# ImIntheMiddle/VATL4Pose-WACV2024

Hardware: AMD Instinct MI355X
Metric: frames/sec pose-infer+uncertainty, 256x192 17-kp (higher is better)
Workload: dtype f32; 1 GPU; SimpleBaseline-R50 256x192 inference + decode + local-peak + THC-L1, 1024-frame synthetic video per GPU; frames_per_gpu=1024, batch=1024, tracks=4, parallelism=frame-sharded x1

## Files before the change

### include/vatl_hip.h

```cpp
#ifndef VATL_HIP_H
#define VATL_HIP_H

#include <stdint.h>

#ifdef __cplusplus
extern "C" {
#endif

#define VATL_VERSION 100
#define VATL_EINVAL  (-1)
#define VATL_ELAUNCH (-2)

int         vatl_version(void);
const char* vatl_last_error(void);

int vatl_flop_meter_begin(void);
int vatl_flop_meter_end(double* direct_flops, double* winograd_flops, int64_t* direct_launches, int64_t* winograd_launches);
#define VATL_ROUTE_NAMES "igemm,igemm_bnbwd,igemm_dma,persistent_1x1,streamk,rows_1x1,bottleneck_chain,stem_pool,halo_3x3," \
                         "winograd,winograd_2h,winograd_bnbwd,winograd_persist,winograd_c32,wgrad,winograd_wgrad,winograd_wgrad_2h," \
                         "winograd_wgrad_table,winograd_f4,winograd_f4_bnbwd,gemm1x1_ring,winograd_deconv43,winograd_s2_43,stem_pool_w1d," \
                         "chain_proj,chain_step"
int vatl_flop_meter_routes(int64_t* counts, int n);


int vatl_nchw_to_nhwc(const float* src, float* dst, int N, int C, int H, int W, int Cpad, void* stream);
int vatl_nhwc_to_nchw(const float* src, float* dst, int N, int C, int H, int W, void* stream);

int vatl_pack_conv_weight(const float* w_oihw, float* w_packed, int Cout, int Cin, int R, int S,
                          int CoutPad, int Spad, int CinPad, void* stream);
int vatl_pack_deconv4x4s2_weight(const float* w_iohw, float* w_packed, int Cin, int Cout, int CoutPad, void* stream);
int64_t vatl_stem_pool_weight_floats(void);
int vatl_pack_stem_pool_weight(const float* w_oihw, float* packed, void* stream);
int vatl_stem_pool_supported(int H, int W);
int vatl_stem7x7s2_pool_fwd(const float* x_nchw, const float* w_packed, const float* scale, const float* bias, float* y_nhwc,
                            int N, int H, int W, void* stream);
int64_t vatl_stem_pool_w1d_weight_floats(void);
int vatl_pack_stem_pool_w1d_weight(const float* w_oihw, float* packed, void* stream);
int vatl_stem_pool_w1d_supported(int H, int W);
int vatl_stem7x7s2_pool_w1d_fwd(const float* x_nchw, const float* w_packed, const float* scale, const float* bias, float* y_nhwc,
                                int N, int H, int W, void* stream);
int64_t vatl_stem3_weight_floats(void);
int vatl_pack_stem3_weight(const float* w_oihw, float* packed, void* stream);
int vatl_stem3x3s2_fwd(const float* x_nchw, const float* w_packed, const float* scale, const float* bias, float* y_nhwc,
                       int N, int H, int W, void* stream);

int vatl_bn_fold(const float* gamma, const float* beta, const float* mean, const float* var, const float* conv_bias,
                 float eps, float* scale, float* bias, int C, void* stream);


int vatl_pack_conv1x1_dual_weight(const float* w1, const float* scale1, const float* bias1, const float* w2, const float* scale2,
                                  const float* bias2, float* out, float* bias, int Cout, int C1, int C2, int CoutPad, void* stream);
int vatl_conv1x1_dual_fwd(const float* a, const float* x, const float* w, const float* bias, float* y, int N, int Ho, int Wo,
                          int C1, int H2, int W2, int C2, int stride2, int Cout, int CoutPad, int relu, void* stream);

int64_t vatl_winograd_c32_weight_floats(void);
int vatl_pack_winograd_c32_weight(const float* w, float* u, void* stream);
int vatl_conv3x3_winograd_c32_supported(int N, int H, int W, int Cin, int Cout);
int vatl_conv3x3_winograd_c32_fwd(const float* x, const float* u, const float* scale, const float* bias, const float* residual, float* y, int N, int H, int W,
                                  int relu, void* stream);

int64_t vatl_winograd_f4_weight_floats(int Cout, int Cin);
int vatl_pack_winograd_f4_weight(const float* w, float* u, int Cout, int Cin, int data_gradient, void* stream);
int vatl_conv3x3_winograd_f4_supported(int N, int H, int W, int Cin, int Cout);
int vatl_conv3x3_winograd_f4_fwd(const float* x, const float* u, const float* scale, const float* bias, const float* residual, float* y, int N, int H, int W,
                                 int Cin, int Cout, int relu, void* stream);
int64_t vatl_winograd_f4_stats_row_blocks(int64_t N, int H, int W);
int vatl_conv3x3_winograd_f4_fwd_stats(const float* x, const float* u, float* y, double* stats, int64_t* row_blocks_used, int N, int H, int W, int Cin, int Cout,
                                       void* stream);
int vatl_conv3x3_winograd_f4_fwd_bnbwd(const float* x, const float* u, const float* residual, float* y, int N, int H, int W, int Cin, int Cout, const float* bn_z,
                                       const float* bn_mask_y, const float* bn_scale, const float* bn_bias, const float* bn_mean, const float* bn_invstd,
                                       double* stats, int64_t* row_blocks_used, void* stream);

int vatl_conv1x1_rows_supported(int K1, int K2, int N, int64_t M);
int vatl_conv1x1_rows_fwd(const float* a, const float* x2, const float* w, const float* scale, const float* bias, const float* residual, float* y,
                          int64_t M, int K1, int K2, int N, int relu, void* stream);

int vatl_bottleneck_chain_supported(int Cmid, int Cout, int Cnext, int64_t M);
int vatl_bottleneck_chain_fwd(const float* a, const float* w3, const float* scale3, const float* bias3, const float* skip, float* t,
                              const float* w1, const float* scale1, const float* bias1, float* y1, int64_t M, int Cmid, int Cout,
                              int Cnext, void* stream);

int vatl_chain_proj_supported(int Cmid, int Cout, int Cnext, int64_t M);
int vatl_chain_proj_fwd(const float* a, const float* x2, const float* w, const float* scale, const float* bias, float* t, const float* w1,
                        const float* scale1, const float* bias1, float* y1, int64_t M, int Cmid, int Cout, int Cnext, int relu, void* stream);
int vatl_chain_step_supported(int Cmid, int Cout, int Cnext, int64_t M);
int vatl_chain_step_fwd(const float* a, const float* w3, const float* scale3, const float* bias3, const float* skip, float* t, const float* w1,
                        const float* scale1, const float* bias1, float* y1, int64_t M, int Cmid, int Cout, int Cnext, void* stream);

int vatl_tune_set(int knob, int value);
int vatl_set_splitk_workspace(float* workspace, int64_t floats);
int vatl_set_splitk_workspace_thread(float* workspace, int64_t floats);
int64_t vatl_streamk_workspace_bytes(void);
int vatl_set_streamk_workspace_thread(void* workspace, int64_t bytes);
int vatl_conv_cout_pad(int Cout);
int vatl_conv2d_fwd(const float* x, const float* w, const float* scale, const float* bias, const float* residual,
                    float* y, int N, int H, int W, int Cin, int Cout, int CoutPad, int R, int S, int stride, int pad,
                    int relu, int out_nchw, void* stream);

int vatl_deconv4x4s2_fwd(const float* x, const float* w, const float* scale, const float* bias, float* y,
                         int N, int H, int W, int Cin, int Cout, int CoutPad, int relu, void* stream);

int vatl_maxpool3x3s2_fwd(const float* x, float* y, int N, int H, int W, int C, void* stream);
int vatl_gap_fwd(const float* x, float* y, int N, int HW, int C, void* stream);

int vatl_pixelshuffle2_fwd(const float* x, float* y, int N, int H, int W, int C, void* stream);
int vatl_se_scale_add_relu(const float* x, const float* gate, const float* residual, float* y, int N, int HW, int C, void* stream);
int vatl_fuse_upsample_add(const float* base, const float* z0, int shift0, const float* z1, int shift1, const float* z2, int shift2,
                           float* y, int N, int H, int W, int C, int relu, void* stream);
int vatl_upsample_nearest_bwd(const float* dy, const float* yact_or_null, float* dz, int N, int H, int W, int C, int shift, void* stream);
int vatl_gap_bwd(const float* dy, float* dx, int N, int HW, int C, void* stream);


int vatl_decode_argmax_affine(const float* hm, const float* bbox, float* coords, float* maxvals, int32_t* idx,
                              int N, int J, int H, int W, void* stream);
int vatl_decode_pose(const float* hm, const float* bbox, float* kpts, int32_t* idx, float* hp, double* pose_score,
                     int N, int J, int H, int W, void* stream);

int vatl_thc_pairs(const float* a, const float* b, int64_t stride_a, int64_t stride_b, float* out,
                   int P, int J, int HW, int norm, void* stream);
int vatl_thc_combine(const float* pair, const uint8_t* is_prev, const uint8_t* is_next, float* thc, int N, void* stream);
// ... 243 lines not shown
```

### vatl4pose-wacv2024_amd/alphapose/models/hip_engine.py

```python
from __future__ import annotations

import time
import weakref

import torch
import torch.nn as nn

import vatl_hip as vh

MAX_CHUNK = 1024



WINOGRAD = True
ROWS_GEMM = True
ROWS_GEMM_K = (128, 256)
WINO_C32 = True
WINO_F4 = True
DECONV_43 = True
S2_43 = True


class _Conv:
    __slots__ = ("w", "u", "u32", "u4", "us2", "wsrc", "wino", "c32", "f4", "s2", "scale", "bias", "cout", "r", "s", "stride", "pad")
# ... 49 lines not shown

    def __init__(self, dc: nn.ConvTranspose2d, bn: nn.BatchNorm2d):
        assert dc.kernel_size == (4, 4) and dc.stride == (2, 2) and dc.padding == (1, 1) and dc.bias is None
        self.cout = dc.weight.shape[1]
        self.u = self.u43 = None
        self.d43 = WINOGRAD and DECONV_43 and dc.weight.shape[0] % 16 == 0 and self.cout % 64 == 0
        self.wsrc = dc.weight.detach() if self.d43 else None
        if WINOGRAD and dc.weight.shape[0] % 16 == 0 and self.cout % 4 == 0:
            self.u = vh.pack_winograd_deconv_weight(dc.weight.detach())
        self.w = vh.pack_deconv_weight(dc.weight.detach())
        self.scale, self.bias = vh.bn_fold(_d(bn.weight), _d(bn.bias), bn.running_mean, bn.running_var, bn.eps)

    def __call__(self, x, relu=True):
        if self.u is not None and not vh.latency_mode():
            if self.d43 and self.u43 is None and vh.deconv4x4s2_winograd43_supported(x.shape[0], x.shape[1], x.shape[2], x.shape[3], self.cout):
                self.u43 = vh.pack_winograd_deconv43_weight(self.wsrc)
            return vh.deconv4x4s2_winograd_fwd(x, self.u, self.scale, self.bias, self.cout, relu, u43=self.u43)
        return vh.deconv4x4s2_fwd(x, self.w, self.scale, self.bias, self.cout, relu)


def _d(p):
    return None if p is None else p.detach()


FUSE_PROJ = True


class _BottleneckPlan:
    def __init__(self, blk):
        self.c1 = _Conv(blk.conv1, blk.bn1)
        self.c2 = _Conv(blk.conv2, blk.bn2)
        self.c3 = _Conv(blk.conv3, blk.bn3)
        self.proj = _Conv(blk.downsample[0], blk.downsample[1]) if blk.downsample is not None else None
        self.dual = None
        if (FUSE_PROJ and self.proj is not None and type(self) is _BottleneckPlan and self.proj.r == 1 and self.c3.cout >= 128
                and blk.conv3.in_channels % 32 == 0 and blk.downsample[0].in_channels % 32 == 0):
            w, b = vh.pack_conv1x1_dual_weight(blk.conv3.weight.detach(), self.c3.scale, self.c3.bias, blk.downsample[0].weight.detach(),
                                               self.proj.scale, self.proj.bias)
            self.dual = (w, b, self.proj.stride)

    def __call__(self, x, out=None, y1=None, nxt=None):
        y = y1 if y1 is not None else self.c1(x, relu=True)
        y = self.c2(y, relu=True)
        return self.tail(y, x, out=out, nxt=nxt)

    def tail(self, y, x, out=None, nxt=None):
        if self.dual is not None:
            if (ROWS_GEMM and self.dual[2] == 1 and y.shape[-1] == 64 and x.shape[-1] == 64 and not vh.latency_mode()
                    and vh.conv1x1_rows_supported(64, 64, self.c3.cout, y.shape[0] * y.shape[1] * y.shape[2])):
                if nxt is not None and FUSE_CHAIN_PROJ and vh.chain_proj_supported(64, self.c3.cout, nxt[0].shape[0], y.shape[0] * y.shape[1] * y.shape[2]):
                    return vh.conv1x1_rows_fwd(y, self.dual[0], None, self.dual[1], self.c3.cout, True, x2=x, out=out, next_conv1=nxt)
                t = vh.conv1x1_rows_fwd(y, self.dual[0], None, self.dual[1], self.c3.cout, True, x2=x, out=out)
            else:
                t = vh.conv1x1_dual_fwd(y, x, self.dual[0], self.dual[1], self.c3.cout, self.dual[2], True, out=out)
        else:
            skip = x if self.proj is None else self.proj(x, relu=False)
            t = self.c3(y, relu=True, residual=skip, out=out)
        return t if nxt is None else (t, None)


FUSE_CHAIN = True
FUSE_CHAIN_PROJ = True
FUSE_CHAIN_STEP = True


def _conv1_of(nxt, cout):
    if (type(nxt) is _BottleneckPlan and (nxt.c1.r, nxt.c1.stride, nxt.c1.pad) == (1, 1, 0) and nxt.c1.scale is not None and nxt.c1.cout == cout
            and not vh.latency_mode()):
        return nxt.c1.w, nxt.c1.scale, nxt.c1.bias
    return None


def _run_blocks(blocks, x, out=None):
    y1 = None
    for k, b in enumerate(blocks):
        last = k == len(blocks) - 1
        o = out if last else None
        if type(b) is not _BottleneckPlan:
            x, y1 = b(x), None
            continue
        nxt = None if last else blocks[k + 1]
        m = x.shape[0] * x.shape[1] * x.shape[2]
        chain = (FUSE_CHAIN and b.proj is None and not vh.latency_mode() and b.c3.scale is not None
                 and vh.bottleneck_chain_supported(b.c3.w.shape[-1], b.c3.cout, 0, m))
        if not chain:
            c1 = _conv1_of(nxt, 64) if b.dual is not None and FUSE_CHAIN_PROJ else None
            x, y1 = b(x, out=o, y1=y1, nxt=c1) if c1 is not None else (b(x, out=o, y1=y1), None)
            continue
        y = b.c2(y1 if y1 is not None else b.c1(x, relu=True), relu=True)
        link, step = _conv1_of(nxt, 64), _conv1_of(nxt, 128) if FUSE_CHAIN_STEP else None
        if link is not None and vh.bottleneck_chain_supported(b.c3.w.shape[-1], b.c3.cout, 64, m):
            x, y1 = vh.bottleneck_chain_fwd(y, b.c3.w, b.c3.scale, b.c3.bias, x, *link, out=o)
        elif step is not None and vh.chain_step_supported(b.c3.w.shape[-1], b.c3.cout, 128, m):
            x, y1 = vh.bottleneck_chain_fwd(y, b.c3.w, b.c3.scale, b.c3.bias, x, out=o, next_stage_conv1=step)
        else:
            x, y1 = vh.bottleneck_chain_fwd(y, b.c3.w, b.c3.scale, b.c3.bias, x, out=o)[0], None
    return x


FUSE_STEM = True
STEM_W1D = True


def _stem_pool_weight(net):
    c = net.conv1
    ok = (FUSE_STEM and tuple(c.weight.shape) == (64, 3, 7, 7) and c.stride == (2, 2) and c.padding == (3, 3) and c.bias is None
          and isinstance(net.maxpool, nn.MaxPool2d) and net.maxpool.kernel_size in (3, (3, 3)) and net.maxpool.stride in (2, (2, 2))
          and net.maxpool.padding in (1, (1, 1)) and not net.maxpool.ceil_mode)
    return vh.pack_stem_pool_weight(c.weight.detach()) if ok else None


class _TrunkPlan:
    def __init__(self, net):
        self.stem = _Conv(net.conv1, net.bn1)
        self.stem_pw = _stem_pool_weight(net)
        self.stem_src, self.stem_u1d = net.conv1.weight.detach(), None
        self.blocks = [_BottleneckPlan(b) for stage in net.stages() for b in stage]
# ... 408 lines not shown
```

### vatl4pose-wacv2024_amd/csrc/common.h

```cpp
#pragma once
#include <hip/hip_runtime.h>
#include <atomic>
#include <cstdarg>
#include <cstdio>
#include <cstdint>

#include "vatl_hip.h"

namespace vatl {

char* err_buf();
int fail(int code, const char* fmt, ...);

void meter_add(int kind, double flops);
enum MeterRoute {
    kRouteIgemm = 0, kRouteIgemmBnBwd, kRouteIgemmDma, kRoutePersistent1x1, kRouteStreamK, kRouteRows, kRouteChain, kRouteStemPool, kRouteHalo,
    kRouteWino, kRouteWino2H, kRouteWinoBnBwd, kRouteWinoPersist, kRouteWinoC32, kRouteWgrad, kRouteWinoWgrad, kRouteWinoWgrad2H,
    kRouteWinoWgradTable, kRouteWinoF4, kRouteWinoF4BnBwd, kRouteGemm1x1Ring, kRouteWinoDeconv43, kRouteWinoS2_43, kRouteStemPoolW1d, kRouteChainProj,
    kRouteChainStep, kRouteCount
};
void meter_route(int route);

inline int check_launch(const char* what) {
    hipError_t e = hipGetLastError();
    if (e != hipSuccess) return fail(VATL_ELAUNCH, "%s: %s", what, hipGetErrorString(e));
    return 0;
}

inline int ensure_dynamic_lds(const void* kern, int bytes, std::atomic<unsigned>& done_mask, const char* what) {
    int d = 0;
    if (hipGetDevice(&d) != hipSuccess) return fail(VATL_ELAUNCH, "%s: no current device", what);
    const unsigned bit = 1u << (d & 31);
    if (done_mask.load(std::memory_order_acquire) & bit) return 0;
    hipError_t e = hipFuncSetAttribute(kern, hipFuncAttributeMaxDynamicSharedMemorySize, bytes);
    if (e != hipSuccess) return fail(VATL_ELAUNCH, "hipFuncSetAttribute(%s): %s", what, hipGetErrorString(e));
    done_mask.fetch_or(bit, std::memory_order_release);
    return 0;
}

__attribute__((visibility("hidden"))) int conv3x3_halo_try(const float* x, const float* w, const float* scale, const float* bias, const float* residual, float* y, int N, int H, int W,
                                                           int Cin, int Cout, int CoutPad, int R, int S, int stride, int pad, int relu, hipStream_t st);

static inline int cdiv(int64_t a, int64_t b) { return (int)((a + b - 1) / b); }

typedef float f32x4 __attribute__((ext_vector_type(4)));

constexpr int kOptBlock = 8192;
typedef float f32x16 __attribute__((ext_vector_type(16)));

__device__ __forceinline__ void lds_barrier() {
    asm volatile("s_waitcnt lgkmcnt(0)" ::: "memory");
    __builtin_amdgcn_s_barrier();
// ... 41 lines not shown
```

### vatl4pose-wacv2024_amd/vatl_hip/__init__.py

```python
from __future__ import annotations

import ctypes as C
import os
import threading as _threading

import torch

_HERE = os.path.dirname(os.path.abspath(__file__))
LIB_PATH = os.environ.get("VATL_HIP_LIB") or os.path.join(_HERE, "libvatl_hip.so")

_p = C.c_void_p
_i = C.c_int
_f = C.c_float
_d = C.c_double
_i64 = C.c_int64

SIGNATURES = {
    "vatl_version": (_i, []),
    "vatl_last_error": (C.c_char_p, []),
    "vatl_flop_meter_begin": (_i, []),
    "vatl_flop_meter_end": (_i, [_p, _p, _p, _p]),
    "vatl_flop_meter_routes": (_i, [_p, _i]),
    "vatl_nchw_to_nhwc": (_i, [_p, _p, _i, _i, _i, _i, _i, _p]),
    "vatl_nhwc_to_nchw": (_i, [_p, _p, _i, _i, _i, _i, _p]),
    "vatl_pack_conv_weight": (_i, [_p, _p, _i, _i, _i, _i, _i, _i, _i, _p]),
    "vatl_pack_deconv4x4s2_weight": (_i, [_p, _p, _i, _i, _i, _p]),
    "vatl_pack_conv1x1_dual_weight": (_i, [_p, _p, _p, _p, _p, _p, _p, _p, _i, _i, _i, _i, _p]),
    "vatl_conv1x1_dual_fwd": (_i, [_p, _p, _p, _p, _p, _i, _i, _i, _i, _i, _i, _i, _i, _i, _i, _i, _p]),
    "vatl_winograd_c32_weight_floats": (_i64, []),
    "vatl_pack_winograd_c32_weight": (_i, [_p, _p, _p]),
    "vatl_conv3x3_winograd_c32_supported": (_i, [_i, _i, _i, _i, _i]),
    "vatl_conv3x3_winograd_c32_fwd": (_i, [_p, _p, _p, _p, _p, _p, _i, _i, _i, _i, _p]),
    "vatl_winograd_f4_weight_floats": (_i64, [_i, _i]),
    "vatl_pack_winograd_f4_weight": (_i, [_p, _p, _i, _i, _i, _p]),
    "vatl_winograd_f4_stats_row_blocks": (_i64, [_i64, _i, _i]),
    "vatl_conv3x3_winograd_f4_fwd_stats": (_i, [_p, _p, _p, _p, _p, _i, _i, _i, _i, _i, _p]),
    "vatl_conv3x3_winograd_f4_fwd_bnbwd": (_i, [_p, _p, _p, _p, _i, _i, _i, _i, _i, _p, _p, _p, _p, _p, _p, _p, _p, _p]),
    "vatl_conv3x3_winograd_f4_supported": (_i, [_i, _i, _i, _i, _i]),
    "vatl_conv3x3_winograd_f4_fwd": (_i, [_p, _p, _p, _p, _p, _p, _i, _i, _i, _i, _i, _i, _p]),
    "vatl_conv1x1_rows_supported": (_i, [_i, _i, _i, _i64]),
    "vatl_conv1x1_rows_fwd": (_i, [_p, _p, _p, _p, _p, _p, _p, _i64, _i, _i, _i, _i, _p]),
    "vatl_bottleneck_chain_supported": (_i, [_i, _i, _i, _i64]),
    "vatl_bottleneck_chain_fwd": (_i, [_p, _p, _p, _p, _p, _p, _p, _p, _p, _p, _i64, _i, _i, _i, _p]),
    "vatl_chain_proj_supported": (_i, [_i, _i, _i, _i64]),
    "vatl_chain_proj_fwd": (_i, [_p, _p, _p, _p, _p, _p, _p, _p, _p, _p, _i64, _i, _i, _i, _i, _p]),
    "vatl_chain_step_supported": (_i, [_i, _i, _i, _i64]),
    "vatl_chain_step_fwd": (_i, [_p, _p, _p, _p, _p, _p, _p, _p, _p, _p, _i64, _i, _i, _i, _p]),
    "vatl_stem_pool_weight_floats": (_i64, []),
    "vatl_pack_stem_pool_weight": (_i, [_p, _p, _p]),
    "vatl_stem_pool_supported": (_i, [_i, _i]),
    "vatl_stem_pool_w1d_weight_floats": (_i64, []),
    "vatl_pack_stem_pool_w1d_weight": (_i, [_p, _p, _p]),
    "vatl_stem_pool_w1d_supported": (_i, [_i, _i]),
    "vatl_stem7x7s2_pool_w1d_fwd": (_i, [_p] * 5 + [_i] * 3 + [_p]),
    "vatl_stem7x7s2_pool_fwd": (_i, [_p, _p, _p, _p, _p, _i, _i, _i, _p]),
    "vatl_stem3_weight_floats": (_i64, []),
    "vatl_pack_stem3_weight": (_i, [_p, _p, _p]),
    "vatl_stem3x3s2_fwd": (_i, [_p, _p, _p, _p, _p, _i, _i, _i, _p]),
    "vatl_bn_fold": (_i, [_p, _p, _p, _p, _p, _f, _p, _p, _i, _p]),
    "vatl_tune_set": (_i, [_i, _i]),
    "vatl_set_splitk_workspace": (_i, [_p, _i64]),
    "vatl_set_splitk_workspace_thread": (_i, [_p, _i64]),
    "vatl_streamk_workspace_bytes": (_i64, []),
    "vatl_set_streamk_workspace_thread": (_i, [_p, _i64]),
    "vatl_conv_cout_pad": (_i, [_i]),
    "vatl_conv2d_fwd": (_i, [_p, _p, _p, _p, _p, _p, _i, _i, _i, _i, _i, _i, _i, _i, _i, _i, _i, _i, _p]),
    "vatl_deconv4x4s2_fwd": (_i, [_p, _p, _p, _p, _p, _i, _i, _i, _i, _i, _i, _i, _p]),
    "vatl_maxpool3x3s2_fwd": (_i, [_p, _p, _i, _i, _i, _i, _p]),
    "vatl_gap_fwd": (_i, [_p, _p, _i, _i, _i, _p]),
    "vatl_pixelshuffle2_fwd": (_i, [_p, _p, _i, _i, _i, _i, _p]),
    "vatl_se_scale_add_relu": (_i, [_p, _p, _p, _p, _i, _i, _i, _p]),
    "vatl_fuse_upsample_add": (_i, [_p, _p, _i, _p, _i, _p, _i, _p, _i, _i, _i, _i, _i, _p]),
    "vatl_upsample_nearest_bwd": (_i, [_p, _p, _p, _i, _i, _i, _i, _i, _p]),
    "vatl_gap_bwd": (_i, [_p, _p, _i, _i, _i, _p]),
    "vatl_decode_argmax_affine": (_i, [_p, _p, _p, _p, _p, _i, _i, _i, _i, _p]),
    "vatl_decode_pose": (_i, [_p, _p, _p, _p, _p, _p, _i, _i, _i, _i, _p]),
    "vatl_thc_pairs": (_i, [_p, _p, _i64, _i64, _p, _i, _i, _i, _i, _p]),
    "vatl_thc_combine": (_i, [_p, _p, _p, _p, _i, _p]),
    "vatl_localpeak_mean": (_i, [_p, _p, _p, _p, _i, _i, _i, _i, _f, _p]),
    "vatl_hybrid_ae_wpu": (_i, [_p, _p, _p, _i, _i, _i, _p, _p, _i, _p]),
# ... 150 lines not shown
    if t.dtype != dtype:
        raise VatlError(f"expected {dtype}, got {t.dtype}")
    if not t.is_contiguous():
        raise VatlError("tensor must be contiguous")
    return t.data_ptr()


def _stream():
    return torch.cuda.current_stream().cuda_stream


_tls = _threading.local()



def nchw_to_nhwc(x: torch.Tensor, cpad: int | None = None) -> torch.Tensor:
    n, c, h, w = x.shape
    cpad = cpad or c
    y = torch.empty((n, h, w, cpad), device=x.device, dtype=torch.float32)
    _check(lib().vatl_nchw_to_nhwc(_ptr(x), _ptr(y), n, c, h, w, cpad, _stream()), "vatl_nchw_to_nhwc")
    return y


def nhwc_to_nchw(x: torch.Tensor) -> torch.Tensor:
    n, h, w, c = x.shape
    y = torch.empty((n, c, h, w), device=x.device, dtype=torch.float32)
    _check(lib().vatl_nhwc_to_nchw(_ptr(x), _ptr(y), n, c, h, w, _stream()), "vatl_nhwc_to_nchw")
    return y



ROUTE_NAMES = ("igemm", "igemm_bnbwd", "igemm_dma", "persistent_1x1", "streamk", "rows_1x1", "bottleneck_chain", "stem_pool", "halo_3x3", "winograd",
               "winograd_2h", "winograd_bnbwd", "winograd_persist", "winograd_c32", "wgrad", "winograd_wgrad", "winograd_wgrad_2h", "winograd_wgrad_table", "winograd_f4", "winograd_f4_bnbwd",
               "gemm1x1_ring", "winograd_deconv43", "winograd_s2_43", "stem_pool_w1d", "chain_proj", "chain_step")


class flop_meter:

    def __enter__(self):
        _check(lib().vatl_flop_meter_begin(), "flop_meter_begin")
        self.direct = self.winograd = self.total = 0.0
        self.direct_launches = self.winograd_launches = 0
        return self

    @staticmethod
    def launches_now() -> int:
        counts = (C.c_int64 * len(ROUTE_NAMES))()
        _check(min(0, lib().vatl_flop_meter_routes(counts, len(ROUTE_NAMES))), "flop_meter_routes")
        return int(sum(counts))

    def __exit__(self, *exc):
        counts = (C.c_int64 * len(ROUTE_NAMES))()
        _check(min(0, lib().vatl_flop_meter_routes(counts, len(ROUTE_NAMES))), "flop_meter_routes")
        self.routes = {n: int(c) for n, c in zip(ROUTE_NAMES, counts)}
        d, w, nd, nw = C.c_double(0), C.c_double(0), C.c_int64(0), C.c_int64(0)
        _check(lib().vatl_flop_meter_end(C.byref(d), C.byref(w), C.byref(nd), C.byref(nw)), "flop_meter_end")
        self.direct, self.winograd, self.total = d.value, w.value, d.value + w.value
        self.direct_launches, self.winograd_launches = nd.value, nw.value
        return False


def tune_set(knob: int, value: int):
    _check(lib().vatl_tune_set(knob, value), "vatl_tune_set")


_splitk_buf = {}

# ... 335 lines not shown
    return bool(lib().vatl_conv3x3s2_winograd43_supported(n, h, w, cin, cout))


def conv2d_fwd(x, w_packed, scale, bias, cout: int, r: int, s: int, stride: int, pad: int, relu: bool,
               residual=None, out_nchw: bool = False, out=None, u_s2=None):
    n, h, w, cin = x.shape
    ho = (h + 2 * pad - r) // stride + 1
    wo = (w + 2 * pad - s) // stride + 1
    shape = (n, cout, ho, wo) if out_nchw else (n, ho, wo, cout)
    y = out if out is not None else torch.empty(shape, device=x.device, dtype=torch.float32)
    if (u_s2 is not None and (r, s, stride, pad) == (3, 3, 2, 1) and residual is None and not out_nchw
            and conv3x3s2_winograd43_supported(n, h, w, cin, cout)):
        _check(lib().vatl_conv3x3s2_winograd43_fwd(_ptr(x), _ptr(u_s2), _ptr(scale), _ptr(bias), _ptr(y), n, h, w, cin, cout, int(relu), _stream()),
               "vatl_conv3x3s2_winograd43_fwd")
        return y
    _check(lib().vatl_conv2d_fwd(_ptr(x), _ptr(w_packed), _ptr(scale), _ptr(bias), _ptr(residual), _ptr(y), n, h, w, cin, cout,
                                 w_packed.shape[0], r, s, stride, pad, int(relu), int(out_nchw), _stream()), "vatl_conv2d_fwd")
    return y


def conv1x1_dual_fwd(a, x, w_packed, bias, cout: int, stride2: int, relu: bool, out=None):
    n, ho, wo, c1 = a.shape
    _, h2, w2, c2 = x.shape
    y = out if out is not None else torch.empty((n, ho, wo, cout), device=a.device, dtype=torch.float32)
    _check(lib().vatl_conv1x1_dual_fwd(_ptr(a), _ptr(x), _ptr(w_packed), _ptr(bias), _ptr(y), n, ho, wo, c1, h2, w2, c2, stride2, cout,
                                       w_packed.shape[0], int(relu), _stream()), "vatl_conv1x1_dual_fwd")
    return y


def conv1x1_rows_supported(k1: int, k2: int, n: int, m: int) -> bool:
    return bool(lib().vatl_conv1x1_rows_supported(k1, k2, n, m))


def conv1x1_rows_fwd(a, w, scale, bias, cout: int, relu: bool, residual=None, x2=None, out=None, next_conv1=None, y1_out=None):
    n, h, w_, k1 = a.shape
    k2 = 0 if x2 is None else x2.shape[-1]
    assert w.numel() >= cout * (k1 + k2) and (x2 is None or tuple(x2.shape[:3]) == (n, h, w_)) and (residual is None or tuple(residual.shape) == (n, h, w_, cout))
    y = out if out is not None else torch.empty((n, h, w_, cout), device=a.device, dtype=torch.float32)
    assert a.is_contiguous() and y.is_contiguous() and (x2 is None or x2.is_contiguous()) and (residual is None or residual.is_contiguous())
    if next_conv1 is not None:
        w1, scale1, bias1 = next_conv1
        cnext = w1.shape[0]
        if x2 is None or k2 != k1 or residual is not None:
            raise VatlError("conv1x1_rows_fwd: next_conv1 goes with the two-source form (a, x2 of 64 channels each) and no residual")
        assert w1.numel() == cnext * cout
        y1 = y1_out if y1_out is not None else torch.empty((n, h, w_, cnext), device=a.device, dtype=torch.float32)
        assert y1.is_contiguous()
        _check(lib().vatl_chain_proj_fwd(_ptr(a), _ptr(x2), _ptr(w), _ptr(scale), _ptr(bias), _ptr(y), _ptr(w1), _ptr(scale1), _ptr(bias1), _ptr(y1),
                                         n * h * w_, k1, cout, cnext, int(relu), _stream()), "vatl_chain_proj_fwd")
        return y, y1
    _check(lib().vatl_conv1x1_rows_fwd(_ptr(a), _ptr(x2), _ptr(w), _ptr(scale), _ptr(bias), _ptr(residual), _ptr(y), n * h * w_, k1, k2, cout, int(relu),
                                       _stream()), "vatl_conv1x1_rows_fwd")
    return y


def bottleneck_chain_supported(cmid: int, cout: int, cnext: int, m: int) -> bool:
    return bool(lib().vatl_bottleneck_chain_supported(cmid, cout, cnext, m))


def chain_proj_supported(cmid: int, cout: int, cnext: int, m: int) -> bool:
    return bool(lib().vatl_chain_proj_supported(cmid, cout, cnext, m))


def chain_step_supported(cmid: int, cout: int, cnext: int, m: int) -> bool:
    return bool(lib().vatl_chain_step_supported(cmid, cout, cnext, m))


def bottleneck_chain_fwd(a, w3, scale3, bias3, skip, w1=None, scale1=None, bias1=None, out=None, y1_out=None, next_stage_conv1=None):
    n, h, w_, cmid = a.shape
    cout = w3.shape[0]
    step = next_stage_conv1 is not None
    if step:
        if w1 is not None:
            raise VatlError("bottleneck_chain_fwd: w1 and next_stage_conv1 are exclusive")
        w1, scale1, bias1 = next_stage_conv1
    cnext = 0 if w1 is None else w1.shape[0]
    assert w3.numel() == cout * cmid and (w1 is None or w1.numel() == cnext * cout) and (skip is None or tuple(skip.shape) == (n, h, w_, cout))
    t = out if out is not None else torch.empty((n, h, w_, cout), device=a.device, dtype=torch.float32)
    assert t.is_contiguous() and a.is_contiguous() and (skip is None or skip.is_contiguous())
    y1 = None if w1 is None else (y1_out if y1_out is not None else torch.empty((n, h, w_, cnext), device=a.device, dtype=torch.float32))
    assert y1 is None or y1.is_contiguous()
    fn, name = (lib().vatl_chain_step_fwd, "vatl_chain_step_fwd") if step else (lib().vatl_bottleneck_chain_fwd, "vatl_bottleneck_chain_fwd")
    _check(fn(_ptr(a), _ptr(w3), _ptr(scale3), _ptr(bias3), _ptr(skip), _ptr(t), _ptr(w1), _ptr(scale1), _ptr(bias1), _ptr(y1),
              n * h * w_, cmid, cout, cnext, _stream()), name)
    return t, y1

# ... 1106 lines not shown
```

Before: 17710 frames/s.

## Fuse bottleneck conv3+residual with next block conv1 in a ring-pipelined kernel

Adds a chain_ring HIP kernel that computes a bottleneck's 128->C 1x1 conv3 with BN, residual add and ReLU, stages each output tile in LDS, and immediately feeds it into the next block's C->128/256 conv1. Weights for both convs are pre-interleaved into one stream and loaded through a 4-slot LDS ring with buffer_load_lds and explicit vmcnt waits. The Python plan routes non-projection bottlenecks with 128-channel mid width onto this path when the chain kernel does not apply. This removes a separate conv1 launch and a re-read of the block output from global memory. In exchange it adds a complex hand-scheduled pipeline with fp32 MFMA and fixed tile sizes, plus a one-time weight packing step.

```diff
diff --git a/include/vatl_hip.h b/include/vatl_hip.h
--- a/include/vatl_hip.h
+++ b/include/vatl_hip.h
@@ -19,7 +19,7 @@
 #define VATL_ROUTE_NAMES "igemm,igemm_bnbwd,igemm_dma,persistent_1x1,streamk,rows_1x1,bottleneck_chain,stem_pool,halo_3x3," \
                          "winograd,winograd_2h,winograd_bnbwd,winograd_persist,winograd_c32,wgrad,winograd_wgrad,winograd_wgrad_2h," \
                          "winograd_wgrad_table,winograd_f4,winograd_f4_bnbwd,gemm1x1_ring,winograd_deconv43,winograd_s2_43,stem_pool_w1d," \
-                         "chain_proj,chain_step"
+                         "chain_proj,chain_step,chain_ring"
 int vatl_flop_meter_routes(int64_t* counts, int n);
 
 
@@ -86,6 +86,12 @@
 int vatl_chain_step_supported(int Cmid, int Cout, int Cnext, int64_t M);
 int vatl_chain_step_fwd(const float* a, const float* w3, const float* scale3, const float* bias3, const float* skip, float* t, const float* w1,
                         const float* scale1, const float* bias1, float* y1, int64_t M, int Cmid, int Cout, int Cnext, void* stream);
+
+int     vatl_chain_ring_supported(int K1, int C, int N2, int64_t M);
+int64_t vatl_chain_ring_stream_floats(int C, int N2);
+int     vatl_pack_chain_ring_stream(const float* w3, const float* w1, float* out, int C, int N2, void* stream);
+int     vatl_chain_ring_fwd(const float* a, const float* wstream, const float* scale3, const float* bias3, const float* skip, float* t, const float* scale1,
+                            const float* bias1, float* y1, int64_t M, int K1, int C, int N2, int relu, void* stream);
 
 int vatl_tune_set(int knob, int value);
 int vatl_set_splitk_workspace(float* workspace, int64_t floats);
diff --git a/vatl4pose-wacv2024_amd/alphapose/models/hip_engine.py b/vatl4pose-wacv2024_amd/alphapose/models/hip_engine.py
--- a/vatl4pose-wacv2024_amd/alphapose/models/hip_engine.py
+++ b/vatl4pose-wacv2024_amd/alphapose/models/hip_engine.py
@@ -105,16 +105,21 @@
         self.c2 = _Conv(blk.conv2, blk.bn2)
         self.c3 = _Conv(blk.conv3, blk.bn3)
         self.proj = _Conv(blk.downsample[0], blk.downsample[1]) if blk.downsample is not None else None
-        self.dual = None
+        self.dual = self.ring_stream = None
         if (FUSE_PROJ and self.proj is not None and type(self) is _BottleneckPlan and self.proj.r == 1 and self.c3.cout >= 128
                 and blk.conv3.in_channels % 32 == 0 and blk.downsample[0].in_channels % 32 == 0):
             w, b = vh.pack_conv1x1_dual_weight(blk.conv3.weight.detach(), self.c3.scale, self.c3.bias, blk.downsample[0].weight.detach(),
                                                self.proj.scale, self.proj.bias)
             self.dual = (w, b, self.proj.stride)
 
-    def __call__(self, x, out=None, y1=None, nxt=None):
+    def __call__(self, x, out=None, y1=None, nxt=None, ring=None):
         y = y1 if y1 is not None else self.c1(x, relu=True)
         y = self.c2(y, relu=True)
+        if ring is not None:
+            if self.ring_stream is None:
+                self.ring_stream = vh.pack_chain_ring_stream(self.c3.w, ring[0])
+            return vh.conv1x1_rows_fwd(y, self.c3.w, self.c3.scale, self.c3.bias, self.c3.cout, True, residual=x, out=out, next_conv1=ring,
+                                       ring_stream=self.ring_stream)
         return self.tail(y, x, out=out, nxt=nxt)
 
     def tail(self, y, x, out=None, nxt=None):
@@ -135,6 +140,7 @@
 FUSE_CHAIN = True
 FUSE_CHAIN_PROJ = True
 FUSE_CHAIN_STEP = True
+FUSE_CHAIN_RING = True
 
 
 def _conv1_of(nxt, cout):
@@ -156,6 +162,11 @@
         m = x.shape[0] * x.shape[1] * x.shape[2]
         chain = (FUSE_CHAIN and b.proj is None and not vh.latency_mode() and b.c3.scale is not None
                  and vh.bottleneck_chain_supported(b.c3.w.shape[-1], b.c3.cout, 0, m))
+        if not chain and FUSE_CHAIN_RING and b.proj is None and b.c3.r == 1 and b.c3.scale is not None and not vh.latency_mode():
+            ring = _conv1_of(nxt, 128) or _conv1_of(nxt, 256)
+            if ring is not None and vh.chain_ring_supported(b.c3.w.shape[-1], b.c3.cout, ring[0].shape[0], m) and ring[0].shape[-1] == b.c3.cout:
+                x, y1 = b(x, out=o, y1=y1, ring=ring)
+                continue
         if not chain:
             c1 = _conv1_of(nxt, 64) if b.dual is not None and FUSE_CHAIN_PROJ else None
             x, y1 = b(x, out=o, y1=y1, nxt=c1) if c1 is not None else (b(x, out=o, y1=y1), None)
diff --git a/vatl4pose-wacv2024_amd/csrc/chain_ring.h b/vatl4pose-wacv2024_amd/csrc/chain_ring.h
--- /dev/null
+++ b/vatl4pose-wacv2024_amd/csrc/chain_ring.h
@@ -0,0 +1,45 @@
+#pragma once
+#include <cstdint>
+
+#if defined(__HIPCC__)
+#define VATL_HD __host__ __device__
+#else
+#define VATL_HD
+#endif
+
+namespace vatl {
+
+constexpr int CR_TM = 64;
+constexpr int CR_STAGE_W = 128 * 16;
+
+VATL_HD inline bool chain_ring_shape_ok(int K1, int C, int N2, int64_t M) {
+    return K1 == 128 && C >= 128 && C <= 4096 && C % 128 == 0 && (N2 == 128 || N2 == 256) && M > 0 && M < (1LL << 30) && (M + 128) * (int64_t)C < (1LL << 30);
+}
+
+VATL_HD inline int chain_ring_period(int N2) { return 8 + 8 * (N2 / 128); }
+VATL_HD inline int64_t chain_ring_stream_floats(int C, int N2) { return (int64_t)(C / 128) * chain_ring_period(N2) * CR_STAGE_W; }
+
+struct ChainRingSrc {
+    int from_w1;
+    int64_t index;
+};
+VATL_HD inline ChainRingSrc chain_ring_stream_src(int64_t o, int C, int N2) {
+    const int period = chain_ring_period(N2);
+    const int64_t stage = o / CR_STAGE_W;
+    const int in = (int)(o - stage * CR_STAGE_W);
+    const int r = in >> 4, pos = (in >> 2) & 3, t = in & 3;
+    const int k = 4 * (pos ^ ((r >> 2) & 3)) + t;
+    const int cb = (int)(stage / period), q = (int)(stage - (int64_t)cb * period);
+    ChainRingSrc s;
+    if (q < 8) {
+        s.from_w1 = 0;
+        s.index = (int64_t)(cb * 128 + r) * 128 + 16 * q + k;
+    } else {
+        const int pass = (q - 8) >> 3, st = (q - 8) & 7;
+        s.from_w1 = 1;
+        s.index = (int64_t)(pass * 128 + r) * C + cb * 128 + 16 * st + k;
+    }
+    return s;
+}
+
+}
diff --git a/vatl4pose-wacv2024_amd/csrc/chain_ring.hip b/vatl4pose-wacv2024_amd/csrc/chain_ring.hip
--- /dev/null
+++ b/vatl4pose-wacv2024_amd/csrc/chain_ring.hip
@@ -0,0 +1,300 @@
+#include "buffer.h"
+#include "chain_ring.h"
+
+#include <atomic>
+#include <type_traits>
+#include <utility>
+
+namespace vatl {
+
+struct ChainRingParams {
+    const float* a;
+    const float* stream;
+    const float* scale3;
+    const float* bias3;
+    const float* res;
+    float* t;
+    const float* scale1;
+    const float* bias1;
+    float* y;
+    int C, ncb, m_tiles, relu3;
+    unsigned a_bytes, t_bytes, y_bytes, s_bytes;
+};
+
+constexpr int CR_SLOT = 64 * 16 + 128 * 16;
+constexpr int CR_TB = 4 * CR_SLOT;
+constexpr int CR_FLOATS = CR_TB + 64 * 128;
+
+template <int N>
+__device__ __forceinline__ void cr_wait_vm() {
+    static_assert(N >= 0 && N <= 63, "the counter has 6 bits");
+    asm volatile("s_waitcnt vmcnt(%0)" ::"n"(N) : "memory");
+}
+
+template <class F, int... I>
+__device__ __forceinline__ void cr_for_each(F& f, std::integer_sequence<int, I...>) {
+    (f(std::integral_constant<int, I>{}), ...);
+}
+
+template <int NP>
+struct CrSched {
+    static constexpr int P = 8 + 8 * NP;
+    static constexpr int D(int q) { return ((q % P + P) % P) < 8 ? 3 : 2; }
+    static constexpr int X(int q) {
+        const int r = (q % P + P) % P;
+        return r == 0 ? 8 : r == 7 ? 32 : 0;
+    }
+    static constexpr int W(int q) { return D(q + 2) + X(q - 2) + X(q - 1); }
+    static constexpr int y_pass(int q) {
+        for (int pp = 0; pp < NP; ++pp) {
+            const int last = 8 * pp + 15;
+            for (int d = 1; d <= 2; ++d)
+                if ((last + d) % P == q) return pp;
+        }
+        return -1;
+    }
+};
+
+template <int NP>
+__global__ __launch_bounds__(256, 2) void chain_ring_kernel(ChainRingParams p) {
+    using S = CrSched<NP>;
+    constexpr int P = S::P;
+    extern __shared__ __attribute__((aligned(16))) float smem[];
+    const int tid = threadIdx.x, lane = tid & 63;
+    const int wave = __builtin_amdgcn_readfirstlane(tid >> 6);
+    const int wm = wave >> 1, wn = wave & 1;
+    const int frow = lane & 31, h = lane >> 5, fsw = (frow >> 2) & 3;
+    const int nblk = gridDim.x, ncb = p.ncb;
+    const unsigned rowb = (unsigned)p.C * 4u;
+    constexpr unsigned rowy = 128u * NP * 4u;
+
+    const __amdgpu_buffer_rsrc_t ar = buf_rsrc(p.a, p.a_bytes);
+    const __amdgpu_buffer_rsrc_t sr = buf_rsrc(p.stream, p.s_bytes);
+    const __amdgpu_buffer_rsrc_t rr = buf_rsrc(p.res ? p.res : p.t, p.res ? p.t_bytes : 0u);
+    const __amdgpu_buffer_rsrc_t tr = buf_rsrc(p.t, p.t_bytes);
+    const __amdgpu_buffer_rsrc_t yr = buf_rsrc(p.y, p.y_bytes);
+
+    const unsigned alane = (unsigned)(wave * 16 + (lane >> 2)) * 512u + (unsigned)((lane & 3) ^ ((lane >> 4) & 3)) * 16u;
+    const unsigned blane = (unsigned)lane * 16u;
+    const unsigned slane = (unsigned)(wm * 32 + (lane >> 4)) * rowb + (unsigned)wn * 256u + (unsigned)(((lane & 15) ^ (lane >> 4)) << 4);
+
+    int ard[2], brd[2], trd[2];
+#pragma unroll
+    for (int g = 0; g < 2; ++g) {
+        ard[g] = (wm * 32 + frow) * 16 + (((2 * g + h) ^ fsw) << 2);
+        brd[g] = 64 * 16 + (wn * 64 + frow) * 16 + (((2 * g + h) ^ fsw) << 2);
+        trd[g] = CR_TB + (wm * 32 + frow) * 64 + (((2 * g + h) ^ (frow & 15)) << 2);
+    }
+    const int twl = CR_TB + wn * 4096 + (wm * 32 + 4 * h) * 64 + ((((frow >> 2) ^ (4 * h)) << 2) | (frow & 3));
+    const unsigned tlane = (unsigned)(wm * 32 + 4 * h) * rowb + (unsigned)(wn * 64 + frow) * 4u;
+    const unsigned ylane = (unsigned)(wm * 32 + 4 * h) * rowy + (unsigned)(wn * 64 + frow) * 4u;
+
+    float sc1[NP][2], bi1[NP][2];
+#pragma unroll
+    for (int pp = 0; pp < NP; ++pp)
+#pragma unroll
+        for (int j = 0; j < 2; ++j) {
+            const int n = pp * 128 + wn * 64 + j * 32 + frow;
+            sc1[pp][j] = p.scale1 ? p.scale1[n] : 1.f;
+            bi1[pp][j] = p.bias1 ? p.bias1[n] : 0.f;
+        }
+    const float lo3 = p.relu3 ? 0.f : -INFINITY;
+
+    f32x16 acc[2], z[NP][2];
+#pragma unroll
+    for (int j = 0; j < 2; ++j)
+#pragma unroll
+        for (int e = 0; e < 16; ++e) {
+            acc[j][e] = 0.f;
+#pragma unroll
+            for (int pp = 0; pp < NP; ++pp) z[pp][j][e] = 0.f;
+        }
+    float sc3[2] = {1.f, 1.f}, bi3[2] = {0.f, 0.f};
+
+    int mt = blockIdx.x, mtn = min(mt + nblk, p.m_tiles), cb = 0;
+    bool y_behind = false;
+
+    auto issue = [&](auto tqc, int slot, int cbq, int tile) {
+        constexpr int TQ = decltype(tqc)::value;
+        float* st = smem + slot * CR_SLOT;
+        if constexpr (TQ < 8)
+            __builtin_amdgcn_raw_ptr_buffer_load_lds(ar, (lds_void*)(st + wave * 256), 16, alane + (unsigned)tile * (64u * 512u), (unsigned)TQ * 64u, 0, 0);
+        const unsigned sbase = (unsigned)(cbq * P + TQ) * (unsigned)(CR_STAGE_W * 4) + (unsigned)wave * 2048u;
+#pragma unroll
+        for (int u = 0; u < 2; ++u)
+            __builtin_amdgcn_raw_ptr_buffer_load_lds(sr, (lds_void*)(st + 64 * 16 + (2 * wave + u) * 256), 16, blane, sbase + (unsigned)u * 1024u, 0, 0);
+    };
+
+    f32x4 fa[2][2], fb[2][2][2];
+    auto read_a = [&](auto qc) {
+        constexpr int Q = decltype(qc)::value, SET = Q & 1, B = Q & 3, G2 = Q >= 8, ST = G2 ? (Q - 8) & 7 : Q;
+#pragma unroll
+        for (int g = 0; g < 2; ++g) {
+            if constexpr (G2) fa[SET][g] = *reinterpret_cast<const f32x4*>(smem + ((trd[g] ^ (16 * (ST & 3))) + 4096 * (ST >> 2)));
+            else fa[SET][g] = *reinterpret_cast<const f32x4*>(smem + ard[g] + B * CR_SLOT);
+        }
+    };
+    auto read_b = [&](auto qc) {
+        constexpr int Q = decltype(qc)::value, SET = Q & 1, B = Q & 3;
+#pragma unroll
+        for (int g = 0; g < 2; ++g)
+#pragma unroll
+            for (int j = 0; j < 2; ++j) fb[SET][g][j] = *reinterpret_cast<const f32x4*>(smem + brd[g] + B * CR_SLOT + j * 32 * 16);
+    };
+
+    auto stage = [&](auto qc) {
+        constexpr int Q = decltype(qc)::value;
+        constexpr int B = Q & 3, SET = Q & 1, G2 = Q >= 8, PASS = G2 ? (Q - 8) >> 3 : 0, ST = G2 ? (Q - 8) & 7 : Q;
+        constexpr int TQ = (Q + 3) % P, WRAP = Q + 3 >= P, DN = S::D(Q + 3), NQ = (Q + 1) % P;
+        constexpr int YP = S::y_pass(Q);
+        (void)ST;
+        if constexpr (YP < 0) cr_wait_vm<S::W(Q)>();
+        else {
+            const bool behind = Q < 2 ? (y_behind && cb == 0) : cb == ncb - 1;
+            if (behind) cr_wait_vm<S::W(Q) + 32>();
+            else cr_wait_vm<S::W(Q)>();
+        }
+        asm volatile("s_waitcnt lgkmcnt(0)" ::: "memory");
+        __builtin_amdgcn_s_barrier();
+        asm volatile("" ::: "memory");
+        if constexpr (Q == 8) read_a(qc);
+        if constexpr (NQ != 8) read_a(std::integral_constant<int, NQ>{});
+        read_b(std::integral_constant<int, NQ>{});
+        {
+            const int cbq = !WRAP ? cb : (cb + 1 == ncb ? 0 : cb + 1);
+            const int tile = (WRAP && cb + 1 == ncb) ? mtn : mt;
+            issue(std::integral_constant<int, TQ>{}, (B + 3) & 3, cbq, tile);
+        }
+        if constexpr (Q == 0) {
+            __builtin_amdgcn_sched_barrier(0);
+            const unsigned sv = slane + (unsigned)(mt * CR_TM) * rowb;
+#pragma unroll
+            for (int u = 0; u < 8; ++u)
+                __builtin_amdgcn_raw_ptr_buffer_load_lds(rr, (lds_void*)(smem + CR_TB + wn * 4096 + (wm * 32 + 4 * u) * 64), 16,
+                                                         (sv + (unsigned)(4 * u) * rowb) ^ (unsigned)((u & 3) * 64), (unsigned)cb * 512u, 0, 0);
+#pragma unroll
+            for (int j = 0; j < 2; ++j) {
+                const int n = cb * 128 + wn * 64 + j * 32 + frow;
+                sc3[j] = p.scale3 ? p.scale3[n] : 1.f;
+                bi3[j] = p.bias3 ? p.bias3[n] : 0.f;
+            }
+            __builtin_amdgcn_sched_barrier(0);
+        }
+#pragma unroll
+        for (int g = 0; g < 2; ++g)
+#pragma unroll
+            for (int tt = 0; tt < 4; ++tt)
+#pragma unroll
+                for (int j = 0; j < 2; ++j) {
+                    if constexpr (G2) z[PASS][j] = __builtin_amdgcn_mfma_f32_32x32x2f32(fa[SET][g][tt], fb[SET][g][j][tt], z[PASS][j], 0, 0, 0);
+                    else acc[j] = __builtin_amdgcn_mfma_f32_32x32x2f32(fa[SET][g][tt], fb[SET][g][j][tt], acc[j], 0, 0, 0);
+                }
+        if constexpr (Q != 0) {
+            __builtin_amdgcn_sched_group_barrier(0x100, (NQ != 8 ? 6 : 4) + (Q == 8 ? 2 : 0), 0);
+#pragma unroll
+            for (int k = 0; k < DN; ++k) {
+                __builtin_amdgcn_sched_group_barrier(0x008, 1, 0);
+                __builtin_amdgcn_sched_group_barrier(0x020, 1, 0);
+            }
+            __builtin_amdgcn_sched_group_barrier(0x008, 16 - DN, 0);
+        }
+        __builtin_amdgcn_sched_barrier(0);
+
+        if constexpr (Q == 7) {
+            unsigned tv = tlane + (unsigned)(mt * CR_TM) * rowb;
+            int twl_ = twl;
+            asm volatile("" : "+v"(twl_), "+v"(tv));
+            auto place = [&](int j, int e) { return smem + ((twl_ + 64 * ((e & 3) + 8 * (e >> 2))) ^ (4 * ((8 * j) ^ (e & 3) ^ (8 * ((e >> 2) & 1))))); };
+            float sk[2][16];
+#pragma unroll
+            for (int j = 0; j < 2; ++j)
+#pragma unroll
+                for (int e = 0; e < 16; ++e) sk[j][e] = *place(j, e);
+#pragma unroll
+            for (int j = 0; j < 2; ++j)
+#pragma unroll
+                for (int e = 0; e < 16; ++e) {
+                    const float v = acc[j][e] * sc3[j] + bi3[j];
+                    const float o = fmaxf(v + sk[j][e], lo3);
+                    *place(j, e) = o;
+                    __builtin_amdgcn_raw_buffer_store_b32(__builtin_bit_cast(unsigned, o), tr, tv + (unsigned)((e & 3) + 8 * (e >> 2)) * rowb,
+                                                          (unsigned)cb * 512u + (unsigned)j * 128u, 0);
+                    acc[j][e] = 0.f;
+                }
+            __builtin_amdgcn_sched_barrier(0);
+        }
+        if constexpr (G2 && ST == 7) {
+            if (cb == ncb - 1) {
+                const unsigned yv = ylane + (unsigned)(mt * CR_TM) * rowy;
+#pragma unroll
+                for (int j = 0; j < 2; ++j)
+#pragma unroll
+                    for (int e = 0; e < 16; ++e) {
+                        const int re = (e & 3) + 8 * (e >> 2);
+                        const float o = fmaxf(z[PASS][j][e] * sc1[PASS][j] + bi1[PASS][j] + 0.f, 0.f);
+                        __builtin_amdgcn_raw_buffer_store_b32(__builtin_bit_cast(unsigned, o), yr, yv + (unsigned)re * rowy, (unsigned)(PASS * 512 + j * 128), 0);
+                        z[PASS][j][e] = 0.f;
+                    }
+            }
+            __builtin_amdgcn_sched_barrier(0);
+        }
+    };
+
+    issue(std::integral_constant<int, 0>{}, 0, 0, mt);
+    issue(std::integral_constant<int, 1>{}, 1, 0, mt);
+    issue(std::integral_constant<int, 2>{}, 2, 0, mt);
+    cr_wait_vm<S::D(1) + S::D(2)>();
+    __builtin_amdgcn_s_barrier();
+    asm volatile("" ::: "memory");
+    read_a(std::integral_constant<int, 0>{});
+    read_b(std::integral_constant<int, 0>{});
+    for (; mt < p.m_tiles; mt = mtn, mtn = min(mtn + nblk, p.m_tiles), y_behind = true)
+        for (cb = 0; cb < ncb; ++cb) cr_for_each(stage, std::make_integer_sequence<int, P>{});
+    asm volatile("s_waitcnt vmcnt(0)" ::: "memory");
+}
+
+__global__ void chain_ring_pack_kernel(const float* __restrict__ w3, const float* __restrict__ w1, float* __restrict__ out, int C, int N2, long long total) {
+    const long long o = (long long)blockIdx.x * blockDim.x + threadIdx.x;
+    if (o >= total) return;
+    const ChainRingSrc s = chain_ring_stream_src(o, C, N2);
+    out[o] = s.from_w1 ? w1[s.index] : w3[s.index];
+}
+
+}
+
+using namespace vatl;
+
+extern "C" int vatl_chain_ring_supported(int K1, int C, int N2, int64_t M) { return chain_ring_shape_ok(K1, C, N2, M) ? 1 : 0; }
+
+extern "C" int64_t vatl_chain_ring_stream_floats(int C, int N2) {
+    return (C >= 128 && C <= 4096 && C % 128 == 0 && (N2 == 128 || N2 == 256)) ? chain_ring_stream_floats(C, N2) : 0;
+}
+
+extern "C" int vatl_pack_chain_ring_stream(const float* w3, const float* w1, float* out, int C, int N2, void* stream) {
+    if (!w3 || !w1 || !out || vatl_chain_ring_stream_floats(C, N2) == 0) return fail(VATL_EINVAL, "pack_chain_ring_stream: bad arguments");
+    const long long total = chain_ring_stream_floats(C, N2);
+    hipLaunchKernelGGL(chain_ring_pack_kernel, dim3((unsigned)((total + 255) / 256)), dim3(256), 0, (hipStream_t)stream, w3, w1, out, C, N2, total);
+    return check_launch("chain_ring_pack");
+}
+
+extern "C" int vatl_chain_ring_fwd(const float* a, const float* wstream, const float* scale3, const float* bias3, const float* skip, float* t, const float* scale1,
+                                   const float* bias1, float* y1, int64_t M, int K1, int C, int N2, int relu, void* stream) {
+    if (!a || !wstream || !t || !y1) return fail(VATL_EINVAL, "chain_ring_fwd: bad arguments");
+    if (!chain_ring_shape_ok(K1, C, N2, M))
+        return fail(VATL_EINVAL, "chain_ring_fwd: serves 128 -> C -> 128 or 256 channels, C a multiple of 128 up to 4096, (M + 128) * C < 2^30");
+    ChainRingParams p{};
+    p.a = a; p.stream = wstream; p.scale3 = scale3; p.bias3 = bias3; p.res = skip; p.t = t; p.scale1 = scale1; p.bias1 = bias1; p.y = y1;
+    p.C = C; p.ncb = C / 128; p.m_tiles = (int)((M + CR_TM - 1) / CR_TM); p.relu3 = relu;
+    p.a_bytes = (unsigned)(M * 128 * 4); p.t_bytes = (unsigned)(M * C * 4); p.y_bytes = (unsigned)(M * N2 * 4);
+    p.s_bytes = (unsigned)(chain_ring_stream_floats(C, N2) * 4);
+    const int smem = CR_FLOATS * (int)sizeof(float);
+    static std::atomic<unsigned> c[2] = {{0}, {0}};
+    void (*kern)(ChainRingParams) = chain_ring_kernel<1>;
+    if (N2 == 256) kern = chain_ring_kernel<2>;
+    if (int rc = ensure_dynamic_lds(reinterpret_cast<const void*>(kern), smem, c[N2 == 256], "chain_ring")) return rc;
+    const int grid = p.m_tiles < 512 ? p.m_tiles : 512;
+    hipLaunchKernelGGL(kern, dim3(grid), dim3(256), smem, (hipStream_t)stream, p);
+    meter_add(0, 2.0 * ((double)p.m_tiles * CR_TM) * (double)C * (double)(128 + N2));
+    meter_route(kRouteChainRing);
+    return check_launch("chain_ring");
+}
diff --git a/vatl4pose-wacv2024_amd/csrc/common.h b/vatl4pose-wacv2024_amd/csrc/common.h
--- a/vatl4pose-wacv2024_amd/csrc/common.h
+++ b/vatl4pose-wacv2024_amd/csrc/common.h
@@ -17,7 +17,7 @@
     kRouteIgemm = 0, kRouteIgemmBnBwd, kRouteIgemmDma, kRoutePersistent1x1, kRouteStreamK, kRouteRows, kRouteChain, kRouteStemPool, kRouteHalo,
     kRouteWino, kRouteWino2H, kRouteWinoBnBwd, kRouteWinoPersist, kRouteWinoC32, kRouteWgrad, kRouteWinoWgrad, kRouteWinoWgrad2H,
     kRouteWinoWgradTable, kRouteWinoF4, kRouteWinoF4BnBwd, kRouteGemm1x1Ring, kRouteWinoDeconv43, kRouteWinoS2_43, kRouteStemPoolW1d, kRouteChainProj,
-    kRouteChainStep, kRouteCount
+    kRouteChainStep, kRouteChainRing, kRouteCount
 };
 void meter_route(int route);
 
diff --git a/vatl4pose-wacv2024_amd/vatl_hip/__init__.py b/vatl4pose-wacv2024_amd/vatl_hip/__init__.py
--- a/vatl4pose-wacv2024_amd/vatl_hip/__init__.py
+++ b/vatl4pose-wacv2024_amd/vatl_hip/__init__.py
@@ -46,6 +46,10 @@
     "vatl_chain_proj_fwd": (_i, [_p, _p, _p, _p, _p, _p, _p, _p, _p, _p, _i64, _i, _i, _i, _i, _p]),
     "vatl_chain_step_supported": (_i, [_i, _i, _i, _i64]),
     "vatl_chain_step_fwd": (_i, [_p, _p, _p, _p, _p, _p, _p, _p, _p, _p, _i64, _i, _i, _i, _p]),
+    "vatl_chain_ring_supported": (_i, [_i, _i, _i, _i64]),
+    "vatl_chain_ring_stream_floats": (_i64, [_i, _i]),
+    "vatl_pack_chain_ring_stream": (_i, [_p, _p, _p, _i, _i, _p]),
+    "vatl_chain_ring_fwd": (_i, [_p, _p, _p, _p, _p, _p, _p, _p, _p, _i64, _i, _i, _i, _i, _p]),
     "vatl_stem_pool_weight_floats": (_i64, []),
     "vatl_pack_stem_pool_weight": (_i, [_p, _p, _p]),
     "vatl_stem_pool_supported": (_i, [_i, _i]),
@@ -262,7 +266,7 @@
 
 ROUTE_NAMES = ("igemm", "igemm_bnbwd", "igemm_dma", "persistent_1x1", "streamk", "rows_1x1", "bottleneck_chain", "stem_pool", "halo_3x3", "winograd",
                "winograd_2h", "winograd_bnbwd", "winograd_persist", "winograd_c32", "wgrad", "winograd_wgrad", "winograd_wgrad_2h", "winograd_wgrad_table", "winograd_f4", "winograd_f4_bnbwd",
-               "gemm1x1_ring", "winograd_deconv43", "winograd_s2_43", "stem_pool_w1d", "chain_proj", "chain_step")
+               "gemm1x1_ring", "winograd_deconv43", "winograd_s2_43", "stem_pool_w1d", "chain_proj", "chain_step", "chain_ring")
 
 
 class flop_meter:
@@ -664,17 +668,33 @@
     return bool(lib().vatl_conv1x1_rows_supported(k1, k2, n, m))
 
 
-def conv1x1_rows_fwd(a, w, scale, bias, cout: int, relu: bool, residual=None, x2=None, out=None, next_conv1=None, y1_out=None):
+def conv1x1_rows_fwd(a, w, scale, bias, cout: int, relu: bool, residual=None, x2=None, out=None, next_conv1=None, y1_out=None, ring_stream=None):
     n, h, w_, k1 = a.shape
     k2 = 0 if x2 is None else x2.shape[-1]
     assert w.numel() >= cout * (k1 + k2) and (x2 is None or tuple(x2.shape[:3]) == (n, h, w_)) and (residual is None or tuple(residual.shape) == (n, h, w_, cout))
     y = out if out is not None else torch.empty((n, h, w_, cout), device=a.device, dtype=torch.float32)
     assert a.is_contiguous() and y.is_contiguous() and (x2 is None or x2.is_contiguous()) and (residual is None or residual.is_contiguous())
+    if next_conv1 is not None and x2 is None and residual is not None:
+        w1, scale1, bias1 = next_conv1
+        cnext = w1.shape[0]
+        assert w1.numel() == cnext * cout
+        y1 = y1_out if y1_out is not None else torch.empty((n, h, w_, cnext), device=a.device, dtype=torch.float32)
+        assert y1.is_contiguous()
+        if not chain_ring_supported(k1, cout, cnext, n * h * w_):
+            conv1x1_rows_fwd(a, w, scale, bias, cout, relu, residual=residual, out=y)
+            return y, conv2d_fwd(y, w1, scale1, bias1, cnext, 1, 1, 1, 0, True, out=y1)
+        if ring_stream is None:
+            ring_stream = pack_chain_ring_stream(w, w1)
+        assert ring_stream.numel() == int(lib().vatl_chain_ring_stream_floats(cout, cnext))
+        _check(lib().vatl_chain_ring_fwd(_ptr(a), _ptr(ring_stream), _ptr(scale), _ptr(bias), _ptr(residual), _ptr(y), _ptr(scale1), _ptr(bias1), _ptr(y1),
+                                         n * h * w_, k1, cout, cnext, int(relu), _stream()), "vatl_chain_ring_fwd")
+        return y, y1
     if next_conv1 is not None:
         w1, scale1, bias1 = next_conv1
         cnext = w1.shape[0]
         if x2 is None or k2 != k1 or residual is not None:
-            raise VatlError("conv1x1_rows_fwd: next_conv1 goes with the two-source form (a, x2 of 64 channels each) and no residual")
+            raise VatlError("conv1x1_rows_fwd: next_conv1 goes with the two-source form (a, x2 of 64 channels each) and no residual, "
+                            "or with the single-source form and a residual")
         assert w1.numel() == cnext * cout
         y1 = y1_out if y1_out is not None else torch.empty((n, h, w_, cnext), device=a.device, dtype=torch.float32)
         assert y1.is_contiguous()
@@ -684,6 +704,21 @@
     _check(lib().vatl_conv1x1_rows_fwd(_ptr(a), _ptr(x2), _ptr(w), _ptr(scale), _ptr(bias), _ptr(residual), _ptr(y), n * h * w_, k1, k2, cout, int(relu),
                                        _stream()), "vatl_conv1x1_rows_fwd")
     return y
+
+
+def chain_ring_supported(k1: int, c: int, n2: int, m: int) -> bool:
+    return bool(lib().vatl_chain_ring_supported(k1, c, n2, m))
+
+
+def pack_chain_ring_stream(w3: torch.Tensor, w1: torch.Tensor) -> torch.Tensor:
+    c, n2 = w3.shape[0], w1.shape[0]
+    total = int(lib().vatl_chain_ring_stream_floats(c, n2))
+    if total == 0 or w3.numel() != c * 128 or w1.numel() != n2 * c:
+        raise VatlError(f"pack_chain_ring_stream: expected [C][128] and [128 or 256][C] filters with C a multiple of 128, got {tuple(w3.shape)} and {tuple(w1.shape)}")
+    assert w3.is_contiguous() and w1.is_contiguous() and w3.dtype == torch.float32 and w1.dtype == torch.float32
+    out = torch.empty(total, device=w3.device, dtype=torch.float32)
+    _check(lib().vatl_pack_chain_ring_stream(_ptr(w3), _ptr(w1), _ptr(out), c, n2, _stream()), "vatl_pack_chain_ring_stream")
+    return out
 
 
 def bottleneck_chain_supported(cmid: int, cout: int, cnext: int, m: int) -> bool:
```

After: 17780 frames/s (median of 6 runs). About the same (+0.4%).
